# JiahaoPlus/EvoWorld

Hardware: AMD Instinct MI355X
Metric: panoramic frames/sec per clip (576x1024x25f, 25 denoise steps) (higher is better)
Workload: dtype f16

## Files before the change

evoworld_amd/ops.py:

```python
import ctypes

import numpy as np
import torch

from . import _lib
from ._lib import GemmArgs

A_DENSE, A_CONV3X3, A_CONVT3 = _lib.EW_A_DENSE, _lib.EW_A_CONV3X3, _lib.EW_A_CONVT3
ACT_NONE, ACT_SILU, ACT_GEGLU, ACT_GELU = _lib.EW_ACT_NONE, _lib.EW_ACT_SILU, _lib.EW_ACT_GEGLU, _lib.EW_ACT_GELU

_zero_pages = {}


def _stream():
    return ctypes.c_void_p(torch.cuda.current_stream().cuda_stream)


def _ptr(t):
    return None if t is None else ctypes.c_void_p(t.data_ptr())


def _call(name, *args):
    _lib.check(getattr(_lib.load(), name)(*args, _stream()), name)

# ... 575 lines not shown
    return x.shape


def im2col3d(x, kernel, stride, pads, out_size, ldk, relu=False, out=None):
    T, H, W, C = _thwc(x, "x")
    rows = out_size[0] * out_size[1] * out_size[2]
    if out is None:
        out = torch.empty(rows, ldk, dtype=torch.float16, device=x.device)
    else:
        _req(out, torch.float16, "out")
        if out.numel() != rows * ldk:
            raise ValueError(f"out holds {out.numel()} values for {rows} rows of {ldk}")
    _call("ew_im2col3d_f16", _ptr(x), _ptr(out), T, H, W, C, *kernel, *stride, *pads, *out_size, ldk, int(bool(relu)))
    return out


def maxpool3d_relu(x, kernel, stride, pads, out_size):
    T, H, W, C = _thwc(x, "x")
    out = torch.empty(*out_size, C, dtype=torch.float16, device=x.device)
    _call("ew_maxpool3d_relu_f16", _ptr(x), _ptr(out), T, H, W, C, *kernel, *stride, *pads, *out_size)
    return out


def i3d_head(x, w, b, out=None):
    T, H, W, C = _thwc(x, "x")
    _req(w, torch.float32, "w"); _req(b, torch.float32, "b")
    if tuple(w.shape) != (400, 1024) or tuple(b.shape) != (400,):
        raise ValueError(f"i3d_head: w {tuple(w.shape)} / b {tuple(b.shape)}: expected [400,1024] and [400]")
    if out is None:
        out = torch.empty(400, dtype=torch.float32, device=x.device)
    else:
        _req(out, torch.float32, "out")
        if out.numel() != 400:
            raise ValueError(f"out holds {out.numel()} values, expected 400")
    ws = torch.empty(_lib.load().ew_i3d_head_workspace_bytes(), dtype=torch.uint8, device=x.device)
    _call("ew_i3d_head", _ptr(x), T, H, W, C, _ptr(w), _ptr(b), _ptr(out), _ptr(ws))
    return out


def frames_resize_aa_norm(frames, table_h, table_w, mean, std, swap_rb=False):
    if frames.dtype == torch.uint8:
        _req(frames, torch.uint8, "frames")
        kind = 1
        F_, H, W, C = frames.shape if frames.ndim == 4 else (0, 0, 0, 0)
    else:
        _req(frames, torch.float32, "frames")
        kind = 2
        F_, C, H, W = frames.shape if frames.ndim == 4 else (0, 0, 0, 0)
    if C != 3:
        raise ValueError(f"frames: expected uint8 [F,H,W,3] or fp32 [F,3,H,W] frames, got {tuple(frames.shape)}")
    args = []
    for name, (first, count, weights) in (("table_h", table_h), ("table_w", table_w)):
        _req(first, torch.int32, f"{name}[0]"); _req(count, torch.int32, f"{name}[1]"); _req(weights, torch.float32, f"{name}[2]")
        if first.ndim != 1 or count.shape != first.shape or weights.ndim != 2 or weights.shape[0] != first.shape[0]:
            raise ValueError(f"{name}: expected (first [n], count [n], weights [n, taps]), got {tuple(first.shape)}, {tuple(count.shape)}, "
                             f"{tuple(weights.shape)}")
        args += [_ptr(first), _ptr(count), _ptr(weights), weights.shape[1]]
    out_h, out_w = table_h[0].shape[0], table_w[0].shape[0]
    out = torch.empty(F_, out_h, out_w, 8, dtype=torch.float16, device=frames.device)
    mean_std = (ctypes.c_float * 6)(*[float(v) for v in mean], *[float(v) for v in std])
    _call("ew_frames_resize_aa_norm_f16", _ptr(frames), kind, _ptr(out), F_, H, W, out_h, out_w, *args, int(bool(swap_rb)), mean_std)
    return out


def avgpool3x3_relu(x):
    n, H, W, C = _thwc(x, "x")
    out = torch.empty_like(x)
    _call("ew_avgpool3x3_relu_f16", _ptr(x), _ptr(out), n, H, W, C)
    return out


def global_avgpool_relu(x):
    n, h, w, C = _thwc(x, "x")
    out = torch.empty(n, C, dtype=torch.float32, device=x.device)
    _call("ew_global_avgpool_relu_f32", _ptr(x), _ptr(out), n, h, w, C)
    return out


def blur_axis(x, kern, axis):
    _req(x, torch.float32, "x"); _req(kern, torch.float32, "kern")
    H, W = x.shape[-2:]
    out = torch.empty_like(x)
    _call("ew_blur_axis_f32", _ptr(x), _ptr(kern), kern.numel(), _ptr(out), x.numel() // (H * W), H, W, axis)
    return out


def bicubic_resize(x, Ho, Wo, scale=None, shift=None):
    _req(x, torch.float32, "x")
    N, C, H, W = x.shape
    out = torch.empty(N, C, Ho, Wo, dtype=torch.float32, device=x.device)
    _call("ew_bicubic_resize_f32", _ptr(x), _ptr(out), N, C, H, W, Ho, Wo, _ptr(scale), _ptr(shift))
    return out


def vit_patchify(x, P, ldk):
    _req(x, torch.float32, "x")
    N, _, S, _ = x.shape
    out = torch.empty(N * (S // P) ** 2, ldk, dtype=torch.float16, device=x.device)
    _call("ew_vit_patchify_f16", _ptr(x), _ptr(out), N, S, P, ldk)
    return out


def attn_small(q, k, v, o, n_seq, S, heads, D, ld, ld_o, scale):
    _call("ew_attn_small_f16", _ptr(q), _ptr(k), _ptr(v), _ptr(o), n_seq, S, heads, D, ld, ld_o, float(scale))
    return o


def ff_pack(w1, b1, w2):
    dev = w1.device
    H2, C = w1.shape
    H = H2 // 2
    assert C == 320 and H == 1280 and tuple(w2.shape) == (C, H)
    nch = H // 32
    c = torch.arange(nch, device=dev)[:, None]
    r = torch.arange(64, device=dev)[None, :]
    j, i = r // 16, r % 16
    hh, vg = j // 2, j % 2
    src = vg * H + 32 * c + 8 * (i // 4) + 4 * hh + (i % 4)
    sl = torch.arange(8, device=dev)
    w1g = w1.float()[src.reshape(-1)].reshape(nch, 64, C // 64, 8, 8)
    perm1 = (sl[None, :] ^ (torch.arange(64, device=dev)[:, None] & 7))
    w1g = torch.gather(w1g, 3, perm1[None, :, None, :, None].expand(nch, 64, C // 64, 8, 8))
    w1p = w1g.permute(0, 2, 1, 3, 4).contiguous().to(torch.float16)
    b1p = b1.float()[src.reshape(-1)].to(torch.float16).contiguous()
    r2 = torch.arange(C, device=dev)
    jj, i2 = r2 // 16, r2 % 16
    col = (jj // 2) * 32 + (i2 // 4) * 8 + (jj % 2) * 4 + (i2 % 4)
    w2g = w2.float()[col].reshape(C, nch, 4, 8)
    gq = torch.tensor([0, 2, 3, 1], device=dev)[(r2 >> 2) & 3]
    perm2 = (torch.arange(4, device=dev)[None, :] ^ gq[:, None])
    w2g = torch.gather(w2g, 2, perm2[:, None, :, None].expand(C, nch, 4, 8))
    w2p = w2g.permute(1, 0, 2, 3).contiguous().to(torch.float16)
    return w1p, b1p, w2p


def ff_geglu320(x, pack, b2, out, *, rowbias=None, rows_per_group=1, ld_rowbias=None, r1=None, r2=None, c_acc=1.0, c_r1=1.0, c_r2=1.0):
    _req(x, torch.float16, "x")
    a = _lib.FfArgs()
    r1h, r1l = _hl(r1)
    r2h, r2l = _hl(r2)
    oh, ol = _hl(out)
    w1p, b1p, w2p = pack
    a.x, a.w1p, a.b1p, a.w2p, a.b2, a.rowbias = _ptr(x), _ptr(w1p), _ptr(b1p), _ptr(w2p), _ptr(b2), _ptr(rowbias)
    a.r1, a.r1_lo, a.r2, a.r2_lo, a.out, a.out_lo = _ptr(r1h), _ptr(r1l), _ptr(r2h), _ptr(r2l), _ptr(oh), _ptr(ol)
    a.zero_page = _ptr(zero_page(x.device))
    a.M, a.C, a.hidden = x.shape[0], x.shape[1], w2p.shape[0] * 32
    a.rows_per_group = rows_per_group
    a.ld_rowbias = ld_rowbias if ld_rowbias is not None else x.shape[1]
    a.c_acc, a.c_r1, a.c_r2 = c_acc, c_r1, c_r2
    _call("ew_ff_geglu320_f16", ctypes.byref(a))
    return out


def pack_conv_weight(w, cpad=None):
    O, I = w.shape[0], w.shape[1]
    wt = w.reshape(O, I, -1).permute(0, 2, 1)
    if cpad:
        wt = torch.nn.functional.pad(wt, (0, cpad - I))
        I = cpad
    taps = wt.shape[1]
    wt = wt.reshape(O, taps, I // 64, 64).permute(0, 2, 1, 3)
    return wt.reshape(O, -1).to(torch.float16).contiguous()
```

evoworld_amd/unet.py:

```python
import math
import os
from collections import OrderedDict
from types import SimpleNamespace

import torch

from . import ops
from ._model import PackedModel, Spec, Weights
from .ops import ACT_GEGLU, ACT_SILU, Res

DEFAULT_CONFIG = dict(
    sample_size=None, in_channels=18, out_channels=4,
    down_block_types=("CrossAttnDownBlockSpatioTemporal",) * 3 + ("DownBlockSpatioTemporal",),
    up_block_types=("UpBlockSpatioTemporal",) + ("CrossAttnUpBlockSpatioTemporal",) * 3,
    block_out_channels=(320, 640, 1280, 1280), addition_time_embed_dim=256,
    projection_class_embeddings_input_dim=768, layers_per_block=2, cross_attention_dim=1024,
    transformer_layers_per_block=1, num_attention_heads=(5, 10, 20, 20), num_frames=25)

CPAD_IN = 64
SPLIT_DUP_LOG2 = 10


def split_in_offsets(in_channels):
    s = (in_channels + 3) // 4 * 4
# ... 28 lines not shown


def _arch(cfg):
    boc = tuple(cfg["block_out_channels"])
    heads = tuple(cfg["num_attention_heads"])
    n = len(boc)
    L = cfg["layers_per_block"]
    res, trs, plan = [], [], []

    def R(prefix, cin, cout, eps):
        d = SimpleNamespace(p=prefix, cin=cin, cout=cout, eps=eps)
        res.append(d)
        return d

    def TR(prefix, ch, nh):
        d = SimpleNamespace(p=prefix, ch=ch, heads=nh)
        trs.append(d)
        return d

    out = boc[0]
    downs = []
    for i in range(n):
        cin, out = out, boc[i]
        last = i == n - 1
        blk = SimpleNamespace(res=[], attn=[], down=None)
        for l in range(L):
            blk.res.append(R(f"down_blocks.{i}.resnets.{l}", cin if l == 0 else out, out, 1e-5 if last else 1e-6))
            if not last:
                blk.attn.append(TR(f"down_blocks.{i}.attentions.{l}", out, heads[i]))
        if not last:
            blk.down = SimpleNamespace(p=f"down_blocks.{i}.downsamplers.0.conv", ch=out)
        downs.append(blk)
    mid = SimpleNamespace(res=[R("mid_block.resnets.0", boc[-1], boc[-1], 1e-5), R("mid_block.resnets.1", boc[-1], boc[-1], 1e-5)],
                          attn=[TR("mid_block.attentions.0", boc[-1], heads[-1])])
    rev, rheads = boc[::-1], heads[::-1]
    ups = []
    out = rev[0]
    for i in range(n):
        prev, out = out, rev[i]
        cin = rev[min(i + 1, n - 1)]
        blk = SimpleNamespace(res=[], attn=[], up=None)
        for l in range(L + 1):
            skip = cin if l == L else out
            rin = prev if l == 0 else out
            r = R(f"up_blocks.{i}.resnets.{l}", rin + skip, out, 1e-6)
            r.split = (rin, skip)
            blk.res.append(r)
            if i > 0:
                blk.attn.append(TR(f"up_blocks.{i}.attentions.{l}", out, rheads[i]))
        if i < n - 1:
            blk.up = SimpleNamespace(p=f"up_blocks.{i}.upsamplers.0.conv", ch=out)
        ups.append(blk)
    return SimpleNamespace(downs=downs, mid=mid, ups=ups, res=res, trs=trs)


def param_spec(cfg):
    spec = Spec()
    lin, conv, norm = spec.lin, spec.conv, spec.norm
    boc = tuple(cfg["block_out_channels"])
    temb = boc[0] * 4
    X = cfg["cross_attention_dim"]

    def resblock(r):
        s, t = r.p + ".spatial_res_block", r.p + ".temporal_res_block"
        norm(s + ".norm1", r.cin); conv(s + ".conv1", r.cout, r.cin, (3, 3)); lin(s + ".time_emb_proj", r.cout, temb)
        norm(s + ".norm2", r.cout); conv(s + ".conv2", r.cout, r.cout, (3, 3))
        if r.cin != r.cout:
            conv(s + ".conv_shortcut", r.cout, r.cin, (1, 1))
        norm(t + ".norm1", r.cout); conv(t + ".conv1", r.cout, r.cout, (3, 1, 1)); lin(t + ".time_emb_proj", r.cout, temb)
        norm(t + ".norm2", r.cout); conv(t + ".conv2", r.cout, r.cout, (3, 1, 1))
        spec.add(r.p + ".time_mixer.mix_factor", (1,), "mix")

    def attn(p, c, ctx):
        lin(p + ".to_q", c, c, False); lin(p + ".to_k", c, ctx or c, False); lin(p + ".to_v", c, ctx or c, False)
        lin(p + ".to_out.0", c, c)

    def ff(p, c):
        lin(p + ".net.0.proj", 8 * c, c); lin(p + ".net.2", c, 4 * c)

    def transformer(t):
        c = t.ch
        norm(t.p + ".norm", c); lin(t.p + ".proj_in", c, c)
        b = t.p + ".transformer_blocks.0"
        norm(b + ".norm1", c); attn(b + ".attn1", c, None); norm(b + ".norm2", c); attn(b + ".attn2", c, X)
        norm(b + ".norm3", c); ff(b + ".ff", c)
        b = t.p + ".temporal_transformer_blocks.0"
        norm(b + ".norm_in", c); ff(b + ".ff_in", c); norm(b + ".norm1", c); attn(b + ".attn1", c, None)
        norm(b + ".norm2", c); attn(b + ".attn2", c, X); norm(b + ".norm3", c); ff(b + ".ff", c)
        lin(t.p + ".time_pos_embed.linear_1", 4 * c, c); lin(t.p + ".time_pos_embed.linear_2", c, 4 * c)
        spec.add(t.p + ".time_mixer.mix_factor", (1,), "mix")
        lin(t.p + ".proj_out", c, c)

    conv("conv_in", boc[0], cfg["in_channels"], (3, 3))
    lin("time_embedding.linear_1", temb, boc[0]); lin("time_embedding.linear_2", temb, temb)
    lin("add_embedding.linear_1", temb, cfg["projection_class_embeddings_input_dim"]); lin("add_embedding.linear_2", temb, temb)
    a = _arch(cfg)
    for blk in a.downs:
        for r in blk.res:
            resblock(r)
        for t in blk.attn:
            transformer(t)
        if blk.down:
            conv(blk.down.p, blk.down.ch, blk.down.ch, (3, 3))
    resblock(a.mid.res[0]); resblock(a.mid.res[1]); transformer(a.mid.attn[0])
    for blk in a.ups:
        for r in blk.res:
            resblock(r)
        for t in blk.attn:
            transformer(t)
        if blk.up:
            conv(blk.up.p, blk.up.ch, blk.up.ch, (3, 3))
    norm("conv_norm_out", boc[0]); conv("conv_out", cfg["out_channels"], boc[0], (3, 3))
    return spec


def random_state_dict(cfg, seed=0, device="cpu"):
    g = torch.Generator(device=device).manual_seed(seed)
    sd = OrderedDict()
    for name, (shape, kind) in param_spec(cfg).items():
        if isinstance(kind, int):
            bound = 1.0 / math.sqrt(kind)
            sd[name] = (torch.rand(shape, generator=g, device=device) * 2 - 1) * bound
        elif kind == "gamma":
            sd[name] = torch.ones(shape, device=device)
        elif kind == "beta":
            sd[name] = torch.zeros(shape, device=device)
        else:
            sd[name] = torch.full(shape, 0.5, device=device)
    return sd


class UNetSpatioTemporalConditionModel(PackedModel):
    DEFAULTS = DEFAULT_CONFIG
    WEIGHT_FILES = ("diffusion_pytorch_model.safetensors", "diffusion_pytorch_model.fp16.safetensors")
    PRETRAINED_KW = ("qkv_fp8",)
    _spec, _random = staticmethod(param_spec), staticmethod(random_state_dict)

    def __init__(self, **config):
        cfg = dict(DEFAULT_CONFIG)
        cfg["qkv_fp8"] = os.environ.get("EW_QKV_FP8", "0") == "1"
        cfg.update(config)
        cfg["qkv_fp8"] = bool(cfg["qkv_fp8"])
        super().__init__(cfg, torch.float16)
        self.arch = _arch(cfg)
        self.add_embedding = SimpleNamespace(linear_1=SimpleNamespace(
            in_features=cfg["projection_class_embeddings_input_dim"]))
        mode = os.environ.get("EW_RESIDUAL", "split")
        self.split_residual = mode != "fp16"
        self.split_heads = mode == "split"
        self.fp8_blocks = []
        self.attn_log2 = True
        self.split_h1 = self.split_heads
        self.fused_ff = 1 if os.environ.get("EW_FUSED_FF", "1") != "0" else 0
        so = int(os.environ.get("EW_SPLIT_OPERANDS", "2"))
        self.split_operands = so != 0
        self.split_acts = so >= 2
        self.in_split = split_in_offsets(cfg["in_channels"]) if self.split_operands else None
        self._pos_cache = {}
        for hd, c in zip(cfg["num_attention_heads"], cfg["block_out_channels"]):
            if c // hd != 64:
                raise ValueError("evoworld_amd attention kernels are specialised to head_dim 64")

    @classmethod
    def _config_from_json(cls, raw):
        return {k: (tuple(v) if isinstance(v, list) else v) for k, v in raw.items() if k in DEFAULT_CONFIG}

    @classmethod
    def from_zeros(cls, device="cuda", **config):
        m = cls(**config)
        return m.load_state_dict(OrderedDict((k, torch.zeros(shape)) for k, (shape, _) in param_spec(m._cfg).items()), device=device)

    def packed_tensors(self):
        out = []

        def walk(v):
            if isinstance(v, torch.Tensor):
                out.append(v)
            elif isinstance(v, dict):
                for n in sorted(v, key=str):
                    walk(v[n])
            elif isinstance(v, (tuple, list)):
                for t in v:
                    walk(t)
        walk(self.w)
        return out

    def broadcast_weights(self, src=0):
        from . import distributed as D
        D.broadcast_tensors(self.packed_tensors(), src=src)
        keys = [k for k in sorted(self.w, key=str) if isinstance(self.w[k], dict) and "mix" in self.w[k]]
        mix = torch.tensor([self.w[k]["mix"] for k in keys], dtype=torch.float64, device=self.device)
        D.broadcast_tensors([mix], src=src)
        for k, v in zip(keys, mix.tolist()):
            self.w[k]["mix"] = v
        self._pos_cache = {}
        return self

    def weights_checksum(self):
        return float(sum(t.double().sum() for t in self.packed_tensors()))

    def to(self, device=None, dtype=None):
        if device is not None and self.w is not None and torch.device(device) != self.device:
            raise NotImplementedError("weights are packed on the device given at load time")
        return self

    def _pack(self, sd):
        f = Weights(sd, self.device)
        f32, h = f.f32, f.h
        self._pos_cache = {}
        W = {}

        def lin2(k, c, acts=False):
            w = f32(k + ".weight")
            if not (self.split_operands and c == self._cfg["block_out_channels"][0]):
                return h(w), h(f32(k + ".bias"))
            w_hi, w_lo = hi_lo(w)
            return h(torch.cat([w_hi, w_hi, w_lo] if acts else [w_hi, w_lo], dim=1)), h(f32(k + ".bias"))

        def geglu(k):
            w, b = f32(k + ".weight"), f32(k + ".bias")
            n = w.shape[0] // 2
            idx = torch.arange(2 * n, device=self.device).reshape(2, n // 16, 16).permute(1, 0, 2).reshape(-1)
            return h(w[idx]), h(b[idx])

        def ff(k, norm, c):
            d = {"norm": f.pair(norm), "up": geglu(k + ".net.0.proj"), "down": f.pair(k + ".net.2")}
            if c == 320 and 4 * c == sd[k + ".net.2.weight"].shape[1]:
                d["pack"] = ops.ff_pack(f32(k + ".net.0.proj.weight"), f32(k + ".net.0.proj.bias"), f32(k + ".net.2.weight"))
            return d

        def fp8(w):
            return ops.quant_rows_fp8(h(w))

        self.fp8_blocks = []
        temb_w, temb_b, self._temb_off = [], [], {}
        off = 0
        for r in self.arch.res:
            s, t = r.p + ".spatial_res_block", r.p + ".temporal_res_block"
            d = {"n1": f.pair(s + ".norm1"), "c1": f.conv(s + ".conv1"), "n2": f.pair(s + ".norm2"), "c2": f.conv(s + ".conv2"),
                 "tn1": f.pair(t + ".norm1"), "t1": f.conv(t + ".conv1"), "tn2": f.pair(t + ".norm2"), "t2": f.conv(t + ".conv2"),
                 "mix": float(torch.sigmoid(f32(r.p + ".time_mixer.mix_factor")).item())}
            if r.cin != r.cout:
                d["sc"] = (h(f32(s + ".conv_shortcut.weight")[:, :, 0, 0]), h(f32(s + ".conv_shortcut.bias")))
            for which in (s, t):
                temb_w.append(f32(which + ".time_emb_proj.weight"))
                temb_b.append(f32(which + ".time_emb_proj.bias"))
                self._temb_off[which] = off
                off += r.cout
            W[r.p] = d
        W["temb"] = (h(torch.cat(temb_w)), h(torch.cat(temb_b)))
        self._temb_total = off

        cv_w, cv_b, self._cv_off = [], [], {}
        off = 0
        for t in self.arch.trs:
            c = t.ch
            use_fp8 = self._cfg["qkv_fp8"] and c % 64 == 0
            if use_fp8:
                self.fp8_blocks.append(t.p)
            d = {"norm": f.pair(t.p + ".norm"), "proj_in": lin2(t.p + ".proj_in", c, self.split_acts), "proj_out": lin2(t.p + ".proj_out", c),
                 "mix": float(torch.sigmoid(f32(t.p + ".time_mixer.mix_factor")).item()),
                 "pe1": f.pair(t.p + ".time_pos_embed.linear_1"), "pe2": f.pair(t.p + ".time_pos_embed.linear_2")}
            for tag, b in (("s", t.p + ".transformer_blocks.0"), ("t", t.p + ".temporal_transformer_blocks.0")):
                q, k_, v = f32(b + ".attn1.to_q.weight"), f32(b + ".attn1.to_k.weight"), f32(b + ".attn1.to_v.weight")
                if tag == "s":
                    d["s_qk"], d["s_v"] = (fp8(torch.cat([q, k_])), fp8(v)) if use_fp8 else (h(torch.cat([q, k_])), h(v))
                else:
                    d["t_qkv"] = fp8(torch.cat([q, k_, v])) if use_fp8 else h(torch.cat([q, k_, v]))
                    d["t_ff_in"] = ff(b + ".ff_in", b + ".norm_in", c)
                d[tag + "_norm1"], d[tag + "_out"] = f.pair(b + ".norm1"), f.pair(b + ".attn1.to_out.0")
                d[tag + "_ff"] = ff(b + ".ff", b + ".norm3", c)
                cv_w.append(f32(b + ".attn2.to_out.0.weight") @ f32(b + ".attn2.to_v.weight"))
                cv_b.append(f32(b + ".attn2.to_out.0.bias"))
                self._cv_off[(t.p, tag)] = off
                off += c
            W[t.p] = d
        W["cv"] = (h(torch.cat(cv_w)), h(torch.cat(cv_b)))
        self._cv_total = off

        for smp in [blk.down for blk in self.arch.downs if blk.down] + [blk.up for blk in self.arch.ups if blk.up]:
            W[smp.p] = f.conv(smp.p)
        if self.in_split:
            W["conv_in"] = (ops.pack_conv_weight(split_conv_in_weight(f32("conv_in.weight"), self.in_split)), h(f32("conv_in.bias")))
        else:
            W["conv_in"] = f.conv("conv_in", CPAD_IN)
        if self.split_operands:
            w_hi, w_lo = hi_lo(f32("conv_out.weight"))
            W["conv_out"] = (ops.pack_conv_weight(torch.cat([w_hi, w_hi, w_lo] if self.split_acts else [w_hi, w_lo], dim=1)), h(f32("conv_out.bias")))
        else:
            W["conv_out"] = f.conv("conv_out")
        W["norm_out"], W["te1"], W["ae1"] = f.pair("conv_norm_out"), f.pair("time_embedding.linear_1"), f.pair("add_embedding.linear_1")
        W["e2"] = (h(torch.cat([f32("time_embedding.linear_2.weight"), f32("add_embedding.linear_2.weight")], dim=1)),
                   h(f32("time_embedding.linear_2.bias") + f32("add_embedding.linear_2.bias")))
        self.w = W

    def _res(self, rows, C, dev, head=False):
        return Res.empty(rows, C, dev, self.split_heads if head else self.split_residual)

    def _lin2(self, x, w, b, out, **kw):
        C = x.shape[-1]
        if w.shape[1] == C:
            return ops.linear(x, w, b, out=out, **kw)
        c2 = w.shape[1] - C
        return ops.gemm(x, w, out, M=x.shape[0], N=w.shape[0], c1=C, lda=C, a2=x, c2=c2, lda2=C, bias=b, **kw)

    def _resblock(self, r, xs, tembs, B, T, H, W_):
        d = self.w[r.p]
        N, HW = B * T, H * W_
        rows = N * HW
        s, t = r.p + ".spatial_res_block", r.p + ".temporal_res_block"
        x1 = xs[0]
        x2 = xs[1] if len(xs) > 1 else None
        dev = x1.hi.device
        tb_s = tembs[:, self._temb_off[s]:]
        tb_t = tembs[:, self._temb_off[t]:]
        hN = ops.groupnorm(xs, *d["n1"], N, HW, r.eps, True, pool=self._gn_pool)
        h1 = self._conv3x3(hN, *d["c1"], N, H, W_, H, W_, rowbias=tb_s, rows_per_group=T * HW,
                           ld_rowbias=self._temb_total, res_out=self.split_h1)
        h2 = ops.groupnorm([h1], *d["n2"], N, HW, r.eps, True, pool=self._gn_pool)
        if "sc" in d:
            sc = self._res(rows, r.cout, dev, head=True)
            c1 = x1.hi.shape[-1]
            c2 = x2.hi.shape[-1] if x2 is not None else 0
            ops.gemm(x1.hi, d["sc"][0], sc, M=rows, N=r.cout, c1=c1, lda=c1, a2=x2.hi if x2 is not None else None, c2=c2,
                     lda2=c2, bias=d["sc"][1])
        else:
            sc = x1
        xsp = self._conv3x3(h2, *d["c2"], N, H, W_, H, W_, r1=sc, ld_r1=r.cout, res_out=True)
        g1 = ops.groupnorm([xsp], *d["tn1"], B, T * HW, r.eps, True, pool=self._gn_pool)
        t1 = self._convt(g1, *d["t1"], B, T, HW, rowbias=tb_t, rows_per_group=T * HW,
                         ld_rowbias=self._temb_total)
        g2 = ops.groupnorm([t1], *d["tn2"], B, T * HW, r.eps, True, pool=self._gn_pool)
        return self._convt(g2, *d["t2"], B, T, HW, r1=xsp, ld_r1=r.cout, c_acc=1.0 - d["mix"], c_r1=1.0,
                           res_out=True)

    def _pos_emb(self, t, B, T):
        key = (t.p, B, T)
        if key not in self._pos_cache:
            d = self.w[t.p]
            sin = ops.sinusoid_embed(torch.arange(T, device=self.device, dtype=torch.float32), T, t.ch)
            e = ops.linear(ops.linear(sin, *d["pe1"], act=ACT_SILU), *d["pe2"])
            self._pos_cache[key] = e.repeat(B, 1).contiguous()
        return self._pos_cache[key]

    def _ff(self, ff, x, out, ln_kw={}, **epi):
        n = ops.layernorm(x, *ff["norm"], **ln_kw)
        if self.fused_ff and "pack" in ff:
            return ops.ff_geglu320(n, ff["pack"], ff["down"][1], out, **epi)
        C = n.shape[-1]
        return ops.linear(ops.linear(n, *ff["up"], act=ACT_GEGLU), *ff["down"], out=out, ld_r1=C, ld_r2=C if "r2" in epi else 0, **epi)

    def _transformer(self, t, x, cvecs, B, T, H, W_):
        d = self.w[t.p]
        C, N, S = t.ch, B * T, H * W_
        rows = N * S
        dev = x.hi.device
        fp8 = isinstance(d["s_qk"], tuple)
        cv_s = cvecs[:, self._cv_off[(t.p, "s")]:]
        cv_t = cvecs[:, self._cv_off[(t.p, "t")]:]
        hn = ops.groupnorm([x], *d["norm"], N, S, 1e-6, False, pool=self._gn_pool, split_out=d["proj_in"][0].shape[1] == 3 * C)
        h = self._lin2(hn, *d["proj_in"], self._res(rows, C, dev, head=True))
        n1 = ops.layernorm(h, *d["s_norm1"])
        prescale = ops.QK_LOG2_PRESCALE if self.attn_log2 else 1.0
        if fp8:
            n1q, n1s = ops.quant_rows_fp8(n1)
            qk = ops.gemm_fp8(n1q, n1s, *d["s_qk"], c_acc=prescale)
            vt = ops.gemm_fp8(*d["s_v"], n1q, n1s)
            del n1q, n1s
        else:
            qk = ops.linear(n1, d["s_qk"], c_acc=prescale)
            vt = torch.empty(C, rows, dtype=torch.float16, device=dev)
            ops.gemm(d["s_v"], n1, vt, M=C, N=rows, c1=C, lda=C)
        ao = torch.empty(rows, C, dtype=torch.float16, device=dev)
        (ops.attn_spatial_log2 if self.attn_log2 else ops.attn_spatial)(qk, qk[:, C:], vt, ao, N, S, t.heads, 2 * C, rows, C)
        del qk, vt
        h = ops.linear(ao, *d["s_out"], out=self._res(rows, C, dev), rowbias=cv_s, rows_per_group=T * S,
                       ld_rowbias=self._cv_total, r1=h, ld_r1=C)
        h = self._ff(d["s_ff"], h, self._res(rows, C, dev), r1=h)
        pos = self._pos_emb(t, B, T)
        hm = self._ff(d["t_ff_in"], h, Res.empty(rows, C, dev, False), dict(addvec=pos, rows_per_group=S), r1=h, rowbias=pos,
                      rows_per_group=S, ld_rowbias=C)
        n1 = ops.layernorm(hm, *d["t_norm1"])
        qkv = ops.gemm_fp8(*ops.quant_rows_fp8(n1), *d["t_qkv"]) if fp8 else ops.linear(n1, d["t_qkv"])
        ops.attn_temporal(qkv, qkv[:, C:], qkv[:, 2 * C:], ao, B, T, S, t.heads, 3 * C, C)
        del qkv
        hm = ops.linear(ao, *d["t_out"], out=Res.empty(rows, C, dev, False), rowbias=cv_t, rows_per_group=T * S,
                        ld_rowbias=self._cv_total, r1=hm, ld_r1=C)
        a = d["mix"]
        hb = self._ff(d["t_ff"], hm, torch.empty(rows, C, dtype=torch.float16, device=dev), c_acc=1.0 - a, r1=hm, c_r1=1.0 - a, r2=h, c_r2=a)
        return self._lin2(hb, *d["proj_out"], self._res(rows, C, dev), r1=x, ld_r1=C)

    def forward_nhwc(self, x, timestep, encoder_hidden_states, added_time_ids, B, T, H, W_, taps=None):
        cfg, Wt = self._cfg, self.w
        dev = x.device
        ops.streamk_init()
        if getattr(self, "_gn_pool", None) is None or self._gn_pool.buf.device != dev:
            self._gn_pool = ops.WorkspacePool(dev)
        self._gn_pool.reset()
        boc = cfg["block_out_channels"]
        N = B * T
        ts = torch.as_tensor(timestep, dtype=torch.float32, device=dev).reshape(-1)
        t_emb = ops.sinusoid_embed(ts, B, boc[0])
        ids = added_time_ids if (added_time_ids.device == dev and added_time_ids.dtype == torch.float32) else added_time_ids.to(device=dev, dtype=torch.float32)
        a_emb = ops.sinusoid_embed(ids.reshape(-1).contiguous(), B * ids.shape[-1], cfg["addition_time_embed_dim"]).reshape(B, -1)
        h1 = ops.linear(t_emb, *Wt["te1"], act=ACT_SILU)
        h2 = ops.linear(a_emb, *Wt["ae1"], act=ACT_SILU)
        td = boc[0] * 4
        semb = torch.empty(B, td, dtype=torch.float16, device=dev)
        ops.gemm(h1, Wt["e2"][0], semb, M=B, N=td, c1=td, lda=td, a2=h2, c2=td, lda2=td, bias=Wt["e2"][1], act=ACT_SILU)
        tembs = ops.linear(semb, *Wt["temb"])
        ehs = encoder_hidden_states.to(device=dev, dtype=torch.float16).reshape(B, -1).contiguous()
        cvecs = ops.linear(ehs, *Wt["cv"])

        h = self._conv3x3(x, *Wt["conv_in"], N, H, W_, H, W_, res_out=True)
        if taps is not None:
            taps["conv_in"] = (h.float(), H, W_)
        skips = [(h, H, W_)]
        for bi, blk in enumerate(self.arch.downs):
            for l, r in enumerate(blk.res):
                h = self._resblock(r, [h], tembs, B, T, H, W_)
                if blk.attn:
                    h = self._transformer(blk.attn[l], h, cvecs, B, T, H, W_)
                skips.append((h, H, W_))
            if blk.down:
                h = self._conv3x3(h.hi, *Wt[blk.down.p], N, H, W_, H // 2, W_ // 2, stride=2, res_out=True)
                H, W_ = H // 2, W_ // 2
                skips.append((h, H, W_))
            if taps is not None:
                taps[f"down{bi}"] = (h.float(), H, W_)
        m = self.arch.mid
        h = self._resblock(m.res[0], [h], tembs, B, T, H, W_)
        h = self._transformer(m.attn[0], h, cvecs, B, T, H, W_)
        h = self._resblock(m.res[1], [h], tembs, B, T, H, W_)
        if taps is not None:
            taps["mid"] = (h.float(), H, W_)
        for bi, blk in enumerate(self.arch.ups):
            for l, r in enumerate(blk.res):
                sk, sh, sw = skips.pop()
                assert (sh, sw) == (H, W_)
                h = self._resblock(r, [h, sk], tembs, B, T, H, W_)
                if blk.attn:
                    h = self._transformer(blk.attn[l], h, cvecs, B, T, H, W_)
            if blk.up:
                h = self._conv3x3(h.hi, *Wt[blk.up.p], N, H, W_, 2 * H, 2 * W_, upsample=1, res_out=True)
                H, W_ = 2 * H, 2 * W_
            if taps is not None:
                taps[f"up{bi}"] = (h.float(), H, W_)
        wco, bco = Wt["conv_out"]
        C0 = h.hi.shape[-1]
        blocks = wco.shape[1] // (9 * C0)
        hn = ops.groupnorm([h], *Wt["norm_out"], N, H * W_, 1e-5, True, pool=self._gn_pool, split_out=blocks == 3)
        return self._conv3x3(hn, wco, bco, N, H, W_, H, W_, x2=hn if blocks > 1 else None, c2=C0 if blocks > 1 else None)

    @torch.no_grad()
    def __call__(self, sample, timestep, encoder_hidden_states, added_time_ids, return_dict=True, taps=None):
        self._require_loaded()
        if sample.ndim != 5 or sample.shape[2] != self._cfg["in_channels"]:
            raise ValueError(f"sample must be [B,T,{self._cfg['in_channels']},h,w], got {tuple(sample.shape)}")
        B, T, C, H, W_ = sample.shape
        if H % 8 or W_ % 8:
            raise ValueError("latent height/width must be multiples of 8 (three stride-2 levels)")
        x = torch.zeros(B * T * H * W_, CPAD_IN, dtype=torch.float16, device=self.device)
        ops.nchw_f32_to_nhwc_f16(sample.to(device=self.device, dtype=torch.float32).reshape(B * T, C, H, W_).contiguous(),
                                 x, CPAD_IN, split=self.in_split)
        eps = self.forward_nhwc(x, timestep, encoder_hidden_states, added_time_ids, B, T, H, W_, taps=taps)
        oc = self._cfg["out_channels"]
        out = ops.nhwc_f16_to_nchw_f32(eps, B * T, oc, H, W_, oc).reshape(B, T, oc, H, W_)
        ops.streamk_check()
        if not return_dict:
            return (out,)
        return SimpleNamespace(sample=out)
```

include/evoworld_hip.h:

```cpp
#ifndef EVOWORLD_HIP_H
#define EVOWORLD_HIP_H
#include <stddef.h>
#include <stdint.h>
#ifdef __cplusplus
extern "C" {
#endif

typedef int ew_status;
#define EW_OK 0
#define EW_ERR_INVALID_ARG (-1)
#define EW_ERR_UNSUPPORTED (-2)
#define EW_ERR_HIP (-3)

#define EW_ABI_VERSION 18
int ew_abi_version(void);
const char* ew_last_error(void);

enum { EW_A_DENSE = 0, EW_A_CONV3X3 = 1, EW_A_CONVT3 = 2 };
enum { EW_ACT_NONE = 0, EW_ACT_SILU = 1, EW_ACT_GEGLU = 2, EW_ACT_GELU = 3  };

typedef struct ew_gemm_args {
    const void* a;
    const void* a2;
    const void* w;
    const void* bias;
    const void* rowbias;
    const void* r1;
    const void* r2;
    void* out;
    const void* zero_page;
    int M, N;
    int c1, c2;
    int lda, lda2;
    int ld_out, ld_r1, ld_r2, ld_rowbias;
    int mode;
    int n_img, h_in, w_in, h_out, w_out, stride, upsample;
    int tB, tT, tP;
    int rows_per_group;
    int act;
    float c_acc, c_r1, c_r2;
    const void* r1_lo;
    const void* r2_lo;
    void* out_lo;
    int conv_shift;
} ew_gemm_args;

ew_status ew_gemm_f16(const ew_gemm_args* args, void* stream);
void ew_set_gemm_generation(int gen);
int ew_get_gemm_generation(void);
const char* ew_gemm_last_kernel(void);
void ew_set_gemm_debug(int flags);
int ew_gemm_streamk_status(void);
ew_status ew_gemm_streamk_init(void* stream);

int ew_set_cu_budget(int n_cus);
int ew_get_cu_budget(void);
void* ew_stream_create_cu_mask(int first_cu, int n_cus);
ew_status ew_stream_destroy(void* stream);

typedef struct ew_ff_args {
    const void* x;
    const void* w1p;
    const void* b1p;
    const void* w2p;
    const void* b2;
    const void* rowbias;
    const void* r1;
    const void* r1_lo;
    const void* r2;
    const void* r2_lo;
    void* out;
    void* out_lo;
    const void* zero_page;
    int M, C, hidden;
    int rows_per_group, ld_rowbias;
    float c_acc, c_r1, c_r2;
} ew_ff_args;
ew_status ew_ff_geglu320_f16(const ew_ff_args* args, void* stream);

size_t ew_groupnorm_workspace_floats(int n_slabs, int rows, int C_tot, int groups);
ew_status ew_groupnorm_stats_f16(const void* x, const void* x_lo, float* ws, int n_slabs, int rows, int C_src, int c_off,
                                 int C_tot, int groups, void* stream);
ew_status ew_groupnorm_finalize(float* ws, int n_slabs, int rows, int C_tot, int groups, void* stream);
ew_status ew_groupnorm_apply_f16(const void* x, const void* x_lo, const float* ws, const void* gamma, const void* beta,
                                 void* y, int n_slabs, int rows, int C_src, int c_off, int C_tot, int groups, float eps,
                                 int silu, void* stream);
ew_status ew_groupnorm_apply_split_f16(const void* x, const void* x_lo, const float* ws, const void* gamma, const void* beta,
                                       void* y, void* y_lo, int ld_y, int n_slabs, int rows, int C_src, int c_off, int C_tot,
                                       int groups, float eps, int silu, void* stream);

ew_status ew_layernorm_f16(const void* x, const void* x_lo, const void* addvec, int rows_per_group, void* x_out,
                           void* x_out_lo, const void* gamma, const void* beta, void* y, int rows, int C, float eps,
                           void* stream);

ew_status ew_attn_spatial_f16(const void* q, const void* k, const void* vt, void* o, int n_seq, int S, int heads,
                              int ld_qk, long long ld_vt, int ld_o, float scale, void* stream);

ew_status ew_attn_spatial_log2_f16(const void* q, const void* k, const void* vt, void* o, int n_seq, int S, int heads,
                                   int ld_qk, long long ld_vt, int ld_o, void* stream);

ew_status ew_attn_temporal_f16(const void* q, const void* k, const void* v, void* o, int B, int T, int S, int heads,
                               int ld, int ld_o, float scale, void* stream);

ew_status ew_nchw_f32_to_nhwc_f16(const float* x, void* y, int N, int C, int H, int W, int ldc, int c_off, float scale,
                                  void* stream);
ew_status ew_nhwc_f16_to_nchw_f32(const void* x, float* y, int N, int C, int H, int W, int ldc, void* stream);
ew_status ew_nchw_f32_to_nhwc_split_f16(const float* x, void* y, int N, int C, int H, int W, int ldc, int c_off, int lo_off,
                                        int dup_off, float scale, void* stream);

ew_status ew_sinusoid_embed_f16(const float* vals, int n_vals, int n_rows, int dim, void* out, void* stream);

ew_status ew_euler_cfg_step(const void* eps, int ld_eps, float* latents, const float* guidance, float sigma,
                            float sigma_next, void* next_in, int cpad, int T, int h, int w, void* stream);
ew_status ew_euler_cfg_step_split(const void* eps, int ld_eps, float* latents, const float* guidance, float sigma,
                                  float sigma_next, void* next_in, int cpad, int lo_off, int dup_off, int T, int h, int w,
                                  void* stream);

ew_status ew_softmax_rows_f16(const void* hi, const void* lo, void* out, long long rows, int cols, long long ld, void* stream);

ew_status ew_time_conv3_f32(const float* x, const float* w, const float* bias, float* y, int B, int T, int C, int HW, void* stream);

ew_status ew_blur_axis_f32(const float* x, const float* kern, int ksize, float* out, long long planes, int H, int W, int axis,
                           void* stream);
ew_status ew_bicubic_resize_f32(const float* x, float* out, int N, int C, int H, int W, int Ho, int Wo, const float* scale,
                                const float* shift, void* stream);
ew_status ew_vit_patchify_f16(const float* x, void* out, int N, int S, int P, int ldk, void* stream);
ew_status ew_attn_small_f16(const void* q, const void* k, const void* v, void* o, int n_seq, int S, int heads, int D, int ld,
                            int ld_o, float scale, void* stream);

ew_status ew_quant_rows_fp8(const void* x, void* q, float* scale, int rows, int K, void* stream);
ew_status ew_gemm_fp8(const void* a, const float* a_scale, const void* w, const float* w_scale, void* out, int M, int N, int K,
                      long long ld_out, float c_acc, void* stream);

ew_status ew_plucker_embed(const float* rays, const float* c2w, float* out, int N, int H, int W, void* stream);

ew_status ew_cube2equi_gather(const uint8_t* faces, int face_channels, const int16_t* lut, uint8_t* pano, int V, int H,
                              int W, int res, void* stream);

ew_status ew_depth_unproject(const float* depth, const float* extr, const float* intr, float* xyz, int S, int H, int W,
                             void* stream);

size_t ew_select_workspace_bytes(void);
ew_status ew_select_kth_f32(const float* x, size_t n, size_t k, void* ws, float* out2, void* stream);
size_t ew_filter_compact_workspace_bytes(size_t n);
ew_status ew_filter_compact(const float* conf, size_t n, float thr, const float* xyz, const float* img, int img_nchw,
                            unsigned hw, float* out_xyz, unsigned* out_rgbx, void* ws, unsigned* total, void* stream);

ew_status ew_splat_cubemap(const float* xyz, size_t npts, const float* w2c, unsigned long long* zbuf, int V, int res,
                           float fx, float fy, float cx, float cy, float z_near, void* stream);
ew_status ew_splat_resolve(const unsigned long long* zbuf, const uint8_t* rgb, int rgb_stride, uint8_t* faces,
                           int face_channels, int V, int res, void* stream);

ew_status ew_equi2pers(const uint8_t* equi, const float* rot, uint8_t* out, int F, int He, int We, int Hp, int Wp,
                       float fov_x_deg, void* stream);

ew_status ew_resize_aa_u8(const uint8_t* src, uint8_t* tmp, uint8_t* dst, const int* kk_h, const int* bounds_h, int ksize_h,
                          const int* kk_v, const int* bounds_v, int ksize_v, int V, int Hi, int Wi, int Ho, int Wo, void* stream);
ew_status ew_u8_hwc_to_f32_chw(const uint8_t* src, float* dst, int V, int H, int W, void* stream);
ew_status ew_f32_chw_to_u8_hwc(const float* src, uint8_t* dst, int V, int H, int W, void* stream);

ew_status ew_pano_yaw_rotate(const void* src, int src_u8, const float* yaw_deg, float* dst, int V, int H, int W, void* stream);

size_t ew_video_metrics_workspace_bytes(int F, int C, int H, int W);
ew_status ew_video_metrics(const void* a, const void* b, int layout, int F, int C, int H, int W, int what, double* sse, double* ssim,
                           void* workspace, void* stream);

size_t ew_video_metrics_ws_workspace_bytes(int F, int C, int H, int W);
ew_status ew_video_metrics_ws(const void* a, const void* b, int layout, int F, int C, int H, int W, int what, const double* row_w,
                              double* wsse, double* wssim, void* workspace, void* stream);

ew_status ew_gt_dump_map_u8(const uint8_t* src, uint8_t* dst, size_t n, void* stream);

ew_status ew_equi2cube_u8(const uint8_t* pano, uint8_t* cross, int V, int H, int W, int interpolation, void* stream);

enum { EW_IM2COL_F16_NHWC = 0, EW_IM2COL_U8_HWC = 1, EW_IM2COL_F32_CHW = 2 };
ew_status ew_im2col_f16(const void* src, int src_kind, void* out, int n_img, int h_in, int w_in, int C, int k, int stride, int pad,
                        int h_out, int w_out, int ldk, int relu, int swap_rb, const float* first_affine, void* stream);
ew_status ew_maxpool3s2_relu_f16(const void* src, void* out, int n_img, int h_in, int w_in, int C, int h_out, int w_out, void* stream);
size_t ew_lpips_head_workspace_bytes(int F, int h, int w, int C);
ew_status ew_lpips_head(const void* fa, const void* fb, const float* lin, const double* wy, const double* wx, int F, int h, int w, int C,
                        double n_out, double* acc, void* workspace, void* stream);

ew_status ew_video_preprocess_f16(const void* src, int src_kind, void* out, int T, int H, int W, int h_resized, int w_resized, int y0, int x0,
                                  int swap_rb, void* stream);
ew_status ew_im2col3d_f16(const void* src, void* out, int t_in, int h_in, int w_in, int C, int kt, int kh, int kw, int st, int sh, int sw,
                          int pt, int ph, int pw, int t_out, int h_out, int w_out, int ldk, int relu, void* stream);
ew_status ew_maxpool3d_relu_f16(const void* src, void* out, int t_in, int h_in, int w_in, int C, int kt, int kh, int kw, int st, int sh, int sw,
                                int pt, int ph, int pw, int t_out, int h_out, int w_out, void* stream);
size_t ew_i3d_head_workspace_bytes(void);
ew_status ew_i3d_head(const void* x, int t_in, int h_in, int w_in, int C, const float* w, const float* b, float* logits, void* workspace,
                      void* stream);

ew_status ew_frames_resize_aa_norm_f16(const void* src, int src_kind, void* out, int F, int H, int W, int out_h, int out_w, const int* y_first,
                                       const int* y_count, const float* y_weights, int y_taps, const int* x_first, const int* x_count,
                                       const float* x_weights, int x_taps, int swap_rb, const float* mean_std, void* stream);
ew_status ew_avgpool3x3_relu_f16(const void* src, void* out, int n_img, int H, int W, int C, void* stream);
ew_status ew_global_avgpool_relu_f32(const void* src, float* out, int n_img, int h, int w, int C, void* stream);

#ifdef __cplusplus
}
#endif
#endif
```

Before: 5.321.

## Fuse temporal attention QKV, softmax and out-projection into one 320-channel kernel

Adds a HIP kernel that, for C=320 temporal transformer blocks, computes the QKV projection, per-pixel temporal attention across frames, the output projection, and the bias/rowbias/residual epilogue in one pass. Weights are prepacked per head and streamed into LDS with double-buffered buffer-to-LDS loads. The goal is to avoid writing and re-reading the QKV and attention-output intermediates in global memory and to save kernel launches. It applies only to the highest-resolution level with non-fp8 weights, and it adds a custom packing layout and a T<=32 limit.

```diff
diff --git a/evoworld_amd/csrc/temporal_block.hip b/evoworld_amd/csrc/temporal_block.hip
--- /dev/null
+++ b/evoworld_amd/csrc/temporal_block.hip
@@ -0,0 +1,287 @@
+#include "gemm_common.h"
+
+namespace {
+
+constexpr int C = 320, HEADS = 5, HD = 64;
+constexpr int NWV = 8, PIX = 4;
+constexpr int QCH = 4, QKS = 5;
+constexpr int Q_ROW = QKS * 32 + 16;
+constexpr int Q_TILE = 3 * HD * Q_ROW;
+constexpr int O_ROW = HD * 2 + 16;
+constexpr int O_TILE = C * O_ROW;
+constexpr int SLOT = O_TILE;
+constexpr int HEAD_BYTES = QCH * Q_TILE + O_TILE;
+constexpr int NCHK = QCH + 1;
+constexpr int REG = 32 * 144;
+constexpr int LDS_W = 0, LDS_X = 2 * SLOT, LDS_B = LDS_X + PIX * 3 * REG, LDS_BYTES = LDS_B + C * 2;
+constexpr int NPIECE_MAX = (O_TILE / 1024 + NWV - 1) / NWV;
+static_assert(Q_TILE % 1024 == 0 && O_TILE % 1024 == 0, "chunk images are whole DMA pieces");
+constexpr float LOG2E = 1.4426950408889634f;
+
+struct TbP {
+    const f16* x;
+    const char* wp;
+    const f16* b_out;
+    const f16* rowbias;
+    const f16* r1;
+    f16* out;
+    int T, S, n_pix, n_tiles, rows_per_group, ld_rowbias;
+    float scale_log2e;
+};
+
+__device__ __forceinline__ float tb_exp2_p32(const f32x16& sacc, float c, float nm, f16x8 (&pf)[2]) {
+    float l = 0.f;
+#pragma unroll
+    for (int g2 = 0; g2 < 2; ++g2)
+#pragma unroll
+        for (int e = 0; e < 8; ++e) {
+            const f16 ph = (f16)__builtin_amdgcn_exp2f(fmaf(sacc[g2 * 8 + e], c, nm));
+            l += (float)ph;
+            pf[g2][e] = ph;
+        }
+    return l;
+}
+
+__global__ __launch_bounds__(64 * NWV, NWV / 4) void tblock320_kernel(const TbP p) {
+    extern __shared__ __attribute__((aligned(16))) char smem[];
+    const int tid = threadIdx.x;
+    const int lane = tid & 63;
+    const int wave = __builtin_amdgcn_readfirstlane(tid >> 6);
+    const unsigned lane16 = (unsigned)lane * 16u;
+    const int pr = wave >> 1, wn = wave & 1;
+    const int lr = lane & 31, lh = lane >> 5;
+
+    const int G = gridDim.x;
+    const int n_my = (p.n_tiles - (int)blockIdx.x + G - 1) / G;
+    if (n_my <= 0) return;
+
+    auto issue = [&](int hh, int kind, int slot) __attribute__((always_inline)) {
+        const int bytes = kind < QCH ? Q_TILE : O_TILE;
+        const __amdgpu_buffer_rsrc_t rd = __builtin_amdgcn_make_buffer_rsrc((void*)(p.wp + (size_t)hh * HEAD_BYTES + kind * Q_TILE), 0, bytes, 0x00020000);
+        char* d = smem + LDS_W + slot * SLOT;
+#pragma unroll
+        for (int k = 0; k < NPIECE_MAX; ++k) {
+            const int off = (wave + NWV * k) * 1024;
+            if ((NWV - 1 + NWV * k) * 1024 < bytes || off < bytes)
+                __builtin_amdgcn_raw_ptr_buffer_load_lds(rd, (lptr_t)(d + off), 16, (int)lane16, off, 0, 0);
+        }
+    };
+    issue(0, 0, 0);
+    if (tid < C / 8) *(f16x8*)(smem + LDS_B + tid * 16) = *(const f16x8*)(p.b_out + tid * 8);
+    ew_wait_vm0_lgkm0();
+    __syncthreads();
+    issue(0, 1, 1);
+
+    const int rdq = (wn * 3 * 32 + lr) * Q_ROW + lh * 16;
+    const int rdo = (wn * 5 * 32 + lr) * O_ROW + lh * 16;
+    char* const regq = smem + LDS_X + pr * (3 * REG);
+    const int wr_x = lr * 144 + (wn * 32 + 4 * lh) * 2;
+    const int rd_x = lr * 144 + lh * 16;
+
+    f16x8 xf[4 * QKS];
+    auto load_x = [&](int tile) __attribute__((always_inline)) {
+        const int pix = min(tile * PIX + pr, p.n_pix - 1);
+        const int b = pix / p.S, s = pix - b * p.S;
+        const long long m = ((long long)b * p.T + min(lr, p.T - 1)) * p.S + s;
+        const f16* xp = p.x + m * C + lh * 16;
+#pragma unroll
+        for (int ks = 0; ks < 4 * QKS; ++ks) xf[ks] = *(const f16x8*)(xp + (ks >> 1) * 32 + (ks & 1) * 8);
+    };
+    load_x((int)blockIdx.x);
+    const bool pad = lr >= p.T;
+    int slot = 0;
+
+    for (int ti = 0; ti < n_my; ++ti) {
+        const int tile = (int)blockIdx.x + ti * G;
+        if (pad) {
+#pragma unroll
+            for (int ks = 0; ks < 4 * QKS; ++ks) xf[ks] = (f16x8){0, 0, 0, 0, 0, 0, 0, 0};
+        }
+        f32x16 acc2[5];
+#pragma unroll
+        for (int u = 0; u < 5; ++u)
+#pragma unroll
+            for (int i = 0; i < 16; ++i) acc2[u][i] = 0.f;
+
+#pragma unroll 1
+        for (int h = 0; h < HEADS; ++h) {
+            const int hn = h + 1 < HEADS ? h + 1 : 0;
+            f32x16 acc1[3];
+#pragma unroll
+            for (int b = 0; b < 3; ++b)
+#pragma unroll
+                for (int i = 0; i < 16; ++i) acc1[b][i] = 0.f;
+#pragma unroll
+            for (int j = 0; j < QCH; ++j) {
+                const char* wb = smem + LDS_W + slot * SLOT + rdq;
+                f16x8 wf[2][3];
+#pragma unroll
+                for (int b = 0; b < 3; ++b) wf[0][b] = *(const f16x8*)(wb + b * (32 * Q_ROW));
+#pragma unroll
+                for (int s = 0; s < QKS; ++s) {
+                    if (s + 1 < QKS) {
+#pragma unroll
+                        for (int b = 0; b < 3; ++b) wf[(s + 1) & 1][b] = *(const f16x8*)(wb + b * (32 * Q_ROW) + (s + 1) * 32);
+                    }
+                    ew_pin();
+#pragma unroll
+                    for (int b = 0; b < 3; ++b) acc1[b] = __builtin_amdgcn_mfma_f32_32x32x16_f16(wf[s & 1][b], xf[j * QKS + s], acc1[b], 0, 0, 0);
+                    ew_pin();
+                }
+                if (j == QCH - 1) {
+#pragma unroll
+                    for (int b = 0; b < 3; ++b)
+#pragma unroll
+                        for (int rq = 0; rq < 4; ++rq) {
+                            f16x4 v4;
+#pragma unroll
+                            for (int e = 0; e < 4; ++e) v4[e] = (f16)acc1[b][rq * 4 + e];
+                            *(f16x4*)(regq + b * REG + wr_x + rq * 16) = v4;
+                        }
+                }
+                ew_wait_vm0_lgkm0();
+                ew_fence();
+                __builtin_amdgcn_s_barrier();
+                ew_fence();
+                if (j + 2 < NCHK) issue(h, j + 2, slot);
+                else issue(hn, j + 2 - NCHK, slot);
+                slot ^= 1;
+            }
+            f16x8 of[4];
+            {
+                f32x16 sacc;
+#pragma unroll
+                for (int i = 0; i < 16; ++i) sacc[i] = 0.f;
+#pragma unroll
+                for (int st = 0; st < 4; ++st) {
+                    const f16x8 qf = *(const f16x8*)(regq + rd_x + st * 32);
+                    const f16x8 kf = *(const f16x8*)(regq + REG + rd_x + st * 32);
+                    sacc = __builtin_amdgcn_mfma_f32_32x32x16_f16(kf, qf, sacc, 0, 0, 0);
+                }
+                float mx = -INFINITY;
+#pragma unroll
+                for (int r = 0; r < 16; ++r) {
+                    const int key = (r & 3) + 8 * (r >> 2) + 4 * lh;
+                    if (key >= p.T) sacc[r] = -INFINITY;
+                    mx = fmaxf(mx, sacc[r]);
+                }
+                mx = fmaxf(mx, __shfl_xor(mx, 32, 64));
+                const float nm = -mx * p.scale_log2e;
+                f16x8 pf[2];
+                float l = tb_exp2_p32(sacc, p.scale_log2e, nm, pf);
+                l += __shfl_xor(l, 32, 64);
+                const float inv = 1.0f / l;
+                const char* regv = regq + 2 * REG;
+#pragma unroll
+                for (int db = 0; db < 2; ++db) {
+                    f32x16 oacc;
+#pragma unroll
+                    for (int i = 0; i < 16; ++i) oacc[i] = 0.f;
+#pragma unroll
+                    for (int g2 = 0; g2 < 2; ++g2) {
+                        f16x8 vf;
+#pragma unroll
+                        for (int e = 0; e < 8; ++e) {
+                            const int key = 16 * g2 + 4 * lh + (e & 3) + 8 * (e >> 2);
+                            vf[e] = *(const f16*)(regv + key * 144 + (db * 32 + lr) * 2);
+                        }
+                        oacc = __builtin_amdgcn_mfma_f32_32x32x16_f16(vf, pf[g2], oacc, 0, 0, 0);
+                    }
+#pragma unroll
+                    for (int s2 = 0; s2 < 2; ++s2)
+#pragma unroll
+                        for (int e = 0; e < 8; ++e) of[db * 2 + s2][e] = (f16)(oacc[s2 * 8 + e] * inv);
+                }
+            }
+            {
+                const char* wb = smem + LDS_W + slot * SLOT + rdo;
+                f16x8 wf[2][4];
+#pragma unroll
+                for (int s = 0; s < 4; ++s) wf[0][s] = *(const f16x8*)(wb + s * 32);
+#pragma unroll
+                for (int u = 0; u < 5; ++u) {
+                    if (u + 1 < 5) {
+#pragma unroll
+                        for (int s = 0; s < 4; ++s) wf[(u + 1) & 1][s] = *(const f16x8*)(wb + (u + 1) * (32 * O_ROW) + s * 32);
+                    }
+                    ew_pin();
+#pragma unroll
+                    for (int s = 0; s < 4; ++s) acc2[u] = __builtin_amdgcn_mfma_f32_32x32x16_f16(wf[u & 1][s], of[s], acc2[u], 0, 0, 0);
+                    ew_pin();
+                }
+                ew_wait_vm0_lgkm0();
+                ew_fence();
+                __builtin_amdgcn_s_barrier();
+                ew_fence();
+                issue(hn, 1, slot);
+                slot ^= 1;
+            }
+        }
+        {
+            const int pix = tile * PIX + pr;
+            const int pc = min(pix, p.n_pix - 1);
+            const int b = pc / p.S, s = pc - b * p.S;
+            const long long m = ((long long)b * p.T + min(lr, p.T - 1)) * p.S + s;
+            const bool valid = pix < p.n_pix && !pad;
+            const int g = (int)m / p.rows_per_group;
+            const f16* r1p = p.r1 + m * C + wn * 160 + lh * 16;
+            const f16* rbp = p.rowbias + (size_t)g * p.ld_rowbias + wn * 160 + lh * 16;
+            const char* bp = smem + LDS_B + (wn * 160 + lh * 16) * 2;
+            f16* op = p.out + m * C + wn * 160 + lh * 16;
+            f16x8 rv[5][2], rb[5][2];
+#pragma unroll
+            for (int u = 0; u < 5; ++u)
+#pragma unroll
+                for (int hf = 0; hf < 2; ++hf) {
+                    rv[u][hf] = *(const f16x8*)(r1p + u * 32 + hf * 8);
+                    rb[u][hf] = *(const f16x8*)(rbp + u * 32 + hf * 8);
+                }
+            ew_pin();
+#pragma unroll
+            for (int u = 0; u < 5; ++u) {
+#pragma unroll
+                for (int hf = 0; hf < 2; ++hf) {
+                    const f16x8 bv = *(const f16x8*)(bp + (u * 32 + hf * 8) * 2);
+                    f16x8 o;
+#pragma unroll
+                    for (int e = 0; e < 8; ++e) o[e] = (f16)((acc2[u][hf * 8 + e] + (float)bv[e] + (float)rb[u][hf][e]) + (float)rv[u][hf][e]);
+                    if (valid) *(f16x8*)(op + u * 32 + hf * 8) = o;
+                }
+                if (u == 1) {
+                    ew_pin();
+                    if (ti + 1 < n_my) load_x(tile + G);
+                    ew_pin();
+                }
+            }
+        }
+    }
+    ew_wait_vm0();
+}
+
+}
+
+extern "C" ew_status ew_temporal_block320_f16(const void* x, const void* wpack, const void* b_out, const void* rowbias, const void* r1,
+                                              void* out, int B, int T, int S, int C_, int heads, int head_dim, int rows_per_group,
+                                              int ld_rowbias, float scale, void* stream) {
+    EW_REQUIRE(x && wpack && b_out && rowbias && r1 && out, "ew_temporal_block320_f16: null pointer");
+    EW_REQUIRE(C_ == C && heads == HEADS && head_dim == HD, "ew_temporal_block320_f16: built for C = 320, 5 heads of 64 (got %d, %d, %d)", C_, heads,
+               head_dim);
+    EW_REQUIRE(T >= 1 && T <= 32, "ew_temporal_block320_f16: needs 1 <= T <= 32 (T=%d)", T);
+    EW_REQUIRE(B > 0 && S > 0 && rows_per_group >= 1, "ew_temporal_block320_f16: bad B / S / rows_per_group");
+    EW_REQUIRE(ld_rowbias >= C && ld_rowbias % 8 == 0, "ew_temporal_block320_f16: ld_rowbias must be >= 320 and a multiple of 8");
+    EW_REQUIRE((((uintptr_t)x | (uintptr_t)wpack | (uintptr_t)b_out | (uintptr_t)rowbias | (uintptr_t)r1 | (uintptr_t)out) & 15) == 0,
+               "ew_temporal_block320_f16: pointers must be 16-byte aligned");
+    EW_REQUIRE((long long)B * S < (1LL << 30) && (long long)B * T * S < (1LL << 31), "ew_temporal_block320_f16: B * T * S too large");
+    TbP p;
+    p.x = (const f16*)x; p.wp = (const char*)wpack; p.b_out = (const f16*)b_out; p.rowbias = (const f16*)rowbias; p.r1 = (const f16*)r1;
+    p.out = (f16*)out;
+    p.T = T; p.S = S; p.n_pix = B * S; p.n_tiles = ew_cdiv(p.n_pix, PIX);
+    p.rows_per_group = rows_per_group; p.ld_rowbias = ld_rowbias;
+    p.scale_log2e = scale * LOG2E;
+    const int ncu = ew_cu_budget();
+    const int grid = p.n_tiles < ncu ? p.n_tiles : ncu;
+    static std::atomic<unsigned long long> mask{0};
+    if (ew_status st = ew_ensure_dynamic_lds((const void*)tblock320_kernel, LDS_BYTES, mask)) return st;
+    hipLaunchKernelGGL(tblock320_kernel, dim3(grid), dim3(64 * NWV), LDS_BYTES, (hipStream_t)stream, p);
+    return ew_check_launch("ew_temporal_block320_f16");
+}
diff --git a/evoworld_amd/ops.py b/evoworld_amd/ops.py
--- a/evoworld_amd/ops.py
+++ b/evoworld_amd/ops.py
@@ -751,6 +751,41 @@
     return out
 
 
+TBLOCK_Q_ROW, TBLOCK_O_ROW = 88, 72
+
+
+def tblock_pack(w_qkv, w_out):
+    dev = w_qkv.device
+    assert tuple(w_qkv.shape) == (960, 320) and tuple(w_out.shape) == (320, 320)
+    ar = lambda n: torch.arange(n, device=dev)
+    h, lh, e = ar(5)[:, None], ar(2)[None, :, None], ar(8)[None, None, :]
+    R = ar(192)[None, :]
+    blk, i = R // 32, R % 32
+    src = 320 * (blk % 3) + 64 * h + 32 * (blk // 3) + i
+    ks = ar(20)[:, None, None]
+    ch = (ks >> 1) * 32 + lh * 16 + (ks & 1) * 8 + e
+    q = w_qkv.float()[src.reshape(-1)][:, ch.reshape(-1)].reshape(5, 192, 4, 80)
+    q = torch.nn.functional.pad(q, (0, TBLOCK_Q_ROW - 80)).permute(0, 2, 1, 3)
+    i2 = ar(320) % 32
+    n = 32 * (ar(320) // 32) + 16 * ((i2 >> 2) & 1) + 4 * (i2 >> 3) + (i2 & 3)
+    s = ar(4)[:, None, None]
+    d = 32 * (s // 2) + 16 * (s % 2) + 8 * (e >> 2) + 4 * lh + (e & 3)
+    col = (64 * h + d.reshape(1, -1)).reshape(-1)
+    o = w_out.float()[n][:, col].reshape(320, 5, 64).permute(1, 0, 2)
+    o = torch.nn.functional.pad(o, (0, TBLOCK_O_ROW - 64))
+    return torch.cat([q.reshape(5, -1), o.reshape(5, -1)], dim=1).to(torch.float16).contiguous()
+
+
+def temporal_block320(x, pack, b_out, out, *, rowbias, rows_per_group, ld_rowbias, r1, B, T, S, C=320, heads=5, scale=0.125):
+    _req(x, torch.float16, "x")
+    r1h, r1l = _hl(r1)
+    oh, ol = _hl(out)
+    assert r1l is None and ol is None, "ew_temporal_block320_f16 takes plain fp16 streams"
+    _call("ew_temporal_block320_f16", _ptr(x), _ptr(pack), _ptr(b_out), _ptr(rowbias), _ptr(r1h), _ptr(oh), B, T, S, C, heads, C // heads,
+          rows_per_group, ld_rowbias, float(scale))
+    return out
+
+
 def pack_conv_weight(w, cpad=None):
     O, I = w.shape[0], w.shape[1]
     wt = w.reshape(O, I, -1).permute(0, 2, 1)
diff --git a/evoworld_amd/unet.py b/evoworld_amd/unet.py
--- a/evoworld_amd/unet.py
+++ b/evoworld_amd/unet.py
@@ -204,6 +204,7 @@
         self.attn_log2 = True
         self.split_h1 = self.split_heads
         self.fused_ff = 1 if os.environ.get("EW_FUSED_FF", "1") != "0" else 0
+        self.fused_tblock = 1 if os.environ.get("EW_FUSED_TBLOCK", "1") != "0" else 0
         so = int(os.environ.get("EW_SPLIT_OPERANDS", "2"))
         self.split_operands = so != 0
         self.split_acts = so >= 2
@@ -319,6 +320,8 @@
                     d["s_qk"], d["s_v"] = (fp8(torch.cat([q, k_])), fp8(v)) if use_fp8 else (h(torch.cat([q, k_])), h(v))
                 else:
                     d["t_qkv"] = fp8(torch.cat([q, k_, v])) if use_fp8 else h(torch.cat([q, k_, v]))
+                    if c == 320 and t.heads == 5 and not use_fp8:
+                        d["t_pack"] = ops.tblock_pack(torch.cat([q, k_, v]), f32(b + ".attn1.to_out.0.weight"))
                     d["t_ff_in"] = ff(b + ".ff_in", b + ".norm_in", c)
                 d[tag + "_norm1"], d[tag + "_out"] = f.pair(b + ".norm1"), f.pair(b + ".attn1.to_out.0")
                 d[tag + "_ff"] = ff(b + ".ff", b + ".norm3", c)
@@ -433,11 +436,15 @@
         hm = self._ff(d["t_ff_in"], h, Res.empty(rows, C, dev, False), dict(addvec=pos, rows_per_group=S), r1=h, rowbias=pos,
                       rows_per_group=S, ld_rowbias=C)
         n1 = ops.layernorm(hm, *d["t_norm1"])
-        qkv = ops.gemm_fp8(*ops.quant_rows_fp8(n1), *d["t_qkv"]) if fp8 else ops.linear(n1, d["t_qkv"])
-        ops.attn_temporal(qkv, qkv[:, C:], qkv[:, 2 * C:], ao, B, T, S, t.heads, 3 * C, C)
-        del qkv
-        hm = ops.linear(ao, *d["t_out"], out=Res.empty(rows, C, dev, False), rowbias=cv_t, rows_per_group=T * S,
-                        ld_rowbias=self._cv_total, r1=hm, ld_r1=C)
+        if self.fused_tblock and "t_pack" in d and T <= 32:
+            hm = ops.temporal_block320(n1, d["t_pack"], d["t_out"][1], Res.empty(rows, C, dev, False), rowbias=cv_t, rows_per_group=T * S,
+                                       ld_rowbias=self._cv_total, r1=hm, B=B, T=T, S=S)
+        else:
+            qkv = ops.gemm_fp8(*ops.quant_rows_fp8(n1), *d["t_qkv"]) if fp8 else ops.linear(n1, d["t_qkv"])
+            ops.attn_temporal(qkv, qkv[:, C:], qkv[:, 2 * C:], ao, B, T, S, t.heads, 3 * C, C)
+            del qkv
+            hm = ops.linear(ao, *d["t_out"], out=Res.empty(rows, C, dev, False), rowbias=cv_t, rows_per_group=T * S,
+                            ld_rowbias=self._cv_total, r1=hm, ld_r1=C)
         a = d["mix"]
         hb = self._ff(d["t_ff"], hm, torch.empty(rows, C, dtype=torch.float16, device=dev), c_acc=1.0 - a, r1=hm, c_r1=1.0 - a, r2=h, c_r2=a)
         return self._lin2(hb, *d["proj_out"], self._res(rows, C, dev), r1=x, ld_r1=C)
diff --git a/include/evoworld_hip.h b/include/evoworld_hip.h
--- a/include/evoworld_hip.h
+++ b/include/evoworld_hip.h
@@ -12,7 +12,7 @@
 #define EW_ERR_UNSUPPORTED (-2)
 #define EW_ERR_HIP (-3)
 
-#define EW_ABI_VERSION 18
+#define EW_ABI_VERSION 19
 int ew_abi_version(void);
 const char* ew_last_error(void);
 
@@ -78,6 +78,10 @@
 } ew_ff_args;
 ew_status ew_ff_geglu320_f16(const ew_ff_args* args, void* stream);
 
+ew_status ew_temporal_block320_f16(const void* x, const void* wpack, const void* b_out, const void* rowbias, const void* r1, void* out,
+                                   int B, int T, int S, int C, int heads, int head_dim, int rows_per_group, int ld_rowbias, float scale,
+                                   void* stream);
+
 size_t ew_groupnorm_workspace_floats(int n_slabs, int rows, int C_tot, int groups);
 ew_status ew_groupnorm_stats_f16(const void* x, const void* x_lo, float* ws, int n_slabs, int rows, int C_src, int c_off,
                                  int C_tot, int groups, void* stream);
```

Result: no change. 5.340 (median of 6 runs) (+0.3%).
